# dschleef/schroedinger

Measured on AMD Instinct MI355X. Metric: Mpix/s IIWT+OBMC decode, 2160p s16, higher is better.
Workload: dtype s16

## Files before the change

### schroedinger_amd/csrc/iiwt_reg.hip

```cpp

#include "schro_hip_internal.h"
#include "iiwt_steps.h"

namespace schro {
namespace {

#define IWT_LOAD8(p) gload < u32x2 > (p)



__device__ __forceinline__ void
coh_store16 (char *p, u32x4 o)
{
  __hip_atomic_store ((SCHRO_GLOBAL uint64_t *) p, (uint64_t) o.x | ((uint64_t) o.y << 32), __ATOMIC_RELAXED, __HIP_MEMORY_SCOPE_AGENT);
  __hip_atomic_store ((SCHRO_GLOBAL uint64_t *) (p + 8), (uint64_t) o.z | ((uint64_t) o.w << 32), __ATOMIC_RELAXED, __HIP_MEMORY_SCOPE_AGENT);
}

typedef short s16x2 __attribute__ ((ext_vector_type (2)));
typedef uint32_t P;

constexpr int kRegRP = 12;
constexpr int kRegUC = 4 * 62;
constexpr int kRegThreads = 256;

// ... 263 lines not shown
  constexpr Step st = filter_step (F, K);
  constexpr int NT = kind_ntaps (st.kind);
  const P y = st.target ? row[0] : row[1];
  P p = lane_prev (y), n = lane_next (y);
  if constexpr (HEDGE) {
    p = is_first ? __builtin_amdgcn_perm (y, y, 0x01000100u) : p;
    n = is_last ? __builtin_amdgcn_perm (y, y, 0x03020302u) : n;
  }
  const P W[6] = { 0u, p, y, n, 0u, 0u };
  P s[NT];
  gather_taps < F, K, 0, 0, NT > (W, s);
  if (st.target)
    row[1] = lift_apply_pk < F, K > (row[1], s);
  else
    row[0] = lift_apply_pk < F, K > (row[0], s);
}

template < int F, bool HEDGE >
__device__ __forceinline__ void
l1_row (P (&row)[2], bool is_first, bool is_last, P & o0, P & o1)
{
  hstep2 < F, 0, HEDGE > (row, is_first, is_last);
  hstep2 < F, 1, HEDGE > (row, is_first, is_last);
  if constexpr (filter_nsteps (F) == 4) {
    hstep2 < F, 2, HEDGE > (row, is_first, is_last);
    hstep2 < F, 3, HEDGE > (row, is_first, is_last);
  }
  constexpr int SH = filter_shift (F);
  const P a = out_round_pk < SH > (row[0]), b = out_round_pk < SH > (row[1]);
  o0 = __builtin_amdgcn_perm (b, a, 0x05040100u);
  o1 = __builtin_amdgcn_perm (b, a, 0x07060302u);
}

template < int F, int RP, int LO, int HI, int LO1, int HI1, bool HEDGE >
__device__ __forceinline__ void
l1_phase (const IwtJob & job, int r0, int c0, int lane, bool is_first, bool is_last, P (&E)[RP][4])
{
  constexpr int H = filter_halo (F), RP1 = RP / 2 + 2 * H;
  static_assert (H % 2 == 0, "level 1 inside level 0 needs an even tile origin");
  P E1[RP1][2], O1[RP1][2];
  const int nr1 = job.h >> 2, nc1 = job.w >> 2;
  const int q0 = (r0 >> 1) - H;
  const uint32_t voff = (uint32_t) clampi ((c0 >> 1) + 2 * lane, 0, nc1 - 2) * 2u;
  constexpr Rng le = load_rows < F, RP1, LO1, HI1 > (0), lo = load_rows < F, RP1, LO1, HI1 > (1);
#pragma unroll
  for (int k = 0; k < RP1; k++) {
    const int r = clampi (q0 + k, 0, nr1 - 1);
    if (k >= le.lo && k <= le.hi) {
      E1[k][0] = gload < uint32_t > ((const char *) job.l1_sb[0] + (size_t) r * job.l1_sb_stride[0] + voff);
      E1[k][1] = gload < uint32_t > ((const char *) job.l1_sb[1] + (size_t) r * job.l1_sb_stride[1] + voff);
    }
    if (k >= lo.lo && k <= lo.hi) {
      O1[k][0] = gload < uint32_t > ((const char *) job.l1_sb[2] + (size_t) r * job.l1_sb_stride[2] + voff);
      O1[k][1] = gload < uint32_t > ((const char *) job.l1_sb[3] + (size_t) r * job.l1_sb_stride[3] + voff);
    }
  }
  vstep < F, 0, RP1, LO1, HI1 > (E1, O1);
  vstep < F, 1, RP1, LO1, HI1 > (E1, O1);
  if constexpr (filter_nsteps (F) == 4) {
    vstep < F, 2, RP1, LO1, HI1 > (E1, O1);
    vstep < F, 3, RP1, LO1, HI1 > (E1, O1);
  }
  constexpr Rng need = load_rows < F, RP, LO, HI > (0);
#pragma unroll
  for (int i = H; i < RP1 - H; i++) {
    const int k = 2 * (i - H);
    if (k >= need.lo && k <= need.hi)
      l1_row < F, HEDGE > (E1[i], is_first, is_last, E[k][0], E[k][1]);
    if (k + 1 >= need.lo && k + 1 <= need.hi)
      l1_row < F, HEDGE > (O1[i], is_first, is_last, E[k + 1][0], E[k + 1][1]);
  }
}

struct NoWait {
  struct Seen { };
  __device__ __forceinline__ Seen ask () const { return Seen (); }
  __device__ __forceinline__ void settle (Seen) const { }
};

template < int F, int RP, int LO, int HI, bool HEDGE, int COH = 0, typename WAIT = NoWait, int LO1 = 0, int HI1 = -1 >
__device__ __forceinline__ void
reg_tile (const IwtJob & job, int r0, int c0, int nr, int nc, int lane, WAIT wait = WAIT ())
{
  constexpr int H = filter_halo (F);
  P E[RP][4], O[RP][4];

  const int cl = c0 + 4 * lane;
  const uint32_t voff = (uint32_t) clampi (cl, 0, nc - 4) * 2u;
  constexpr Rng le = load_rows < F, RP, LO, HI > (0), lo = load_rows < F, RP, LO, HI > (1);
  const int l_lo = (max (0, -c0) + 3) >> 2, l_hi = min (63, ((nc - c0) >> 2) - 1);
  const bool is_first = lane == l_lo, is_last = lane == l_hi;
  if constexpr ((COH & 8) != 0) {
    l1_phase < F, RP, LO, HI, LO1, HI1, HEDGE > (job, r0, c0, lane, is_first, is_last, E);
    __builtin_amdgcn_sched_barrier (0);
  }
  const auto seen = wait.ask ();
#pragma unroll
  for (int k = 0; k < RP; k++) {
    const int r = clampi (r0 + k, 0, nr - 1);
    if (k >= le.lo && k <= le.hi) {
      const u32x2 hl = IWT_LOAD8 ((const char *) job.sb[1] + (size_t) r * job.sb_stride[1] + voff);
      E[k][2] = hl.x;
      E[k][3] = hl.y;
    }
    if (k >= lo.lo && k <= lo.hi) {
      const u32x2 lh = IWT_LOAD8 ((const char *) job.sb[2] + (size_t) r * job.sb_stride[2] + voff);
      const u32x2 hh = IWT_LOAD8 ((const char *) job.sb[3] + (size_t) r * job.sb_stride[3] + voff);
      O[k][0] = lh.x;
      O[k][1] = lh.y;
      O[k][2] = hh.x;
      O[k][3] = hh.y;
    }
  }
  wait.settle (seen);
  if constexpr ((COH & 8) == 0) {
#pragma unroll
    for (int k = 0; k < RP; k++) {
      const int r = clampi (r0 + k, 0, nr - 1);
      if (k >= le.lo && k <= le.hi) {
        const u32x2 ll = IWT_LOAD8 ((const char *) job.sb[0] + (size_t) r * job.sb_stride[0] + voff);
        E[k][0] = ll.x;
        E[k][1] = ll.y;
      }
    }
  }

  vstep < F, 0, RP, LO, HI > (E, O);
  vstep < F, 1, RP, LO, HI > (E, O);
  if constexpr (filter_nsteps (F) == 4) {
    vstep < F, 2, RP, LO, HI > (E, O);
    vstep < F, 3, RP, LO, HI > (E, O);
  }

  constexpr int LH = (COH & 8) != 0 ? l1_lane_halo (F) : 1;
  const bool store_lane = lane >= max (l_lo, LH) && lane <= min (l_hi, 63 - LH);
  if constexpr ((COH & 4) != 0) {
    const int x = 2 * cl, y0 = 2 * (r0 + H);
    const int nx = store_lane ? clampi (job.out_w - x, 0, 8) : 0;
    const bool full = nx == 8;
    const bool any_ragged = __builtin_amdgcn_readfirstlane ((int) (__ballot (nx > 0 && nx < 8) != 0)) != 0;
    const int xa = nx > 0 ? x : 0;
    char *dst = (char *) job.dst + (size_t) y0 *job.dst_stride + xa;
    const bool has_pred = job.pred != nullptr;
    const uint8_t *pp = job.pred + xa;
    const u32x2 k128 = (u32x2) { 0x80808080u, 0x80808080u };
    auto fetch = [&](int i, int odd) {
      const int row = min (y0 + 2 * (i - H) + odd, job.out_h - 1);
      return has_pred ? __builtin_nontemporal_load ((const SCHRO_GLOBAL u32x2 *) (pp + (size_t) row * job.pred_stride)) : k128;
    };
    constexpr int NPAIR = RP - 2 * H;
    constexpr int AHEAD = cmin (NPAIR, 4), RAMP = 2;
    u32x2 pr[NPAIR][2];
    __builtin_amdgcn_sched_barrier (0);
#pragma unroll
    for (int j = 0; j < AHEAD; j++) {
      pr[j][0] = fetch (H + j, 0);
      pr[j][1] = fetch (H + j, 1);
    }
    __builtin_amdgcn_sched_barrier (0);
#pragma unroll
    for (int i = H; i < RP - H; i++) {
      const int j = i - H;
      const int y = y0 + 2 * j;
      const Combine c0 = { pr[j][0], y < job.out_h, full, any_ragged, nx }, c1 = { pr[j][1], y + 1 < job.out_h, full, any_ragged, nx };
      finish_row < F, HEDGE, COH > (E[i], is_first, is_last, store_lane, dst, c0);
      finish_row < F, HEDGE, COH > (O[i], is_first, is_last, store_lane, dst + job.dst_stride, c1);
      dst += 2 * (size_t) job.dst_stride;
#pragma unroll
      for (int t = 0; t < RAMP; t++) {
        const int nj = AHEAD + RAMP * j + t;
        if (nj < NPAIR) {
          pr[nj][0] = fetch (H + nj, 0);
          pr[nj][1] = fetch (H + nj, 1);
        }
      }
      __builtin_amdgcn_sched_barrier (0);
    }
  } else {
    char *dst = (char *) job.dst + (size_t) (2 * (r0 + H)) * job.dst_stride + (size_t) cl * 4;
    const Combine none = { (u32x2) { 0u, 0u }, false, false, false, 0 };
#pragma unroll
    for (int i = H; i < RP - H; i++) {
      finish_row < F, HEDGE, COH > (E[i], is_first, is_last, store_lane, dst, none);
      finish_row < F, HEDGE, COH > (O[i], is_first, is_last, store_lane, dst + job.dst_stride, none);
      dst += 2 * (size_t) job.dst_stride;
    }
  }
}

template < int F, int RP, int N, int COH, typename WAIT >
__device__ __forceinline__ void
reg_tile_bottom (int nout, const IwtJob & job, int r0, int c0, int nr, int nc, int lane, WAIT wait)
{
  if constexpr (N >= 1) {
    if (nout == N)
      reg_tile < F, RP, 0, RP - 1 - N, true, COH, WAIT > (job, r0, c0, nr, nc, lane, wait);
    else
      reg_tile_bottom < F, RP, N - 1, COH, WAIT > (nout, job, r0, c0, nr, nc, lane, wait);
  }
}

template < int F, int RP >
__device__ __forceinline__ int
reg_tile_r0 (int ty, int nr)
{
  constexpr int H = filter_halo (F), UR = RP - 2 * H;
  int r0 = ty * UR - H;
  if (r0 + H + UR > nr)
    r0 = nr - UR - H;
  return r0;
}

template < int F, int RP, int COH, typename WAIT = NoWait >
__device__ __forceinline__ void
reg_tile_at (const IwtJob & job, int tx, int ty, int lane, WAIT wait = WAIT ())
{
  constexpr int H = filter_halo (F);
  const int nr = job.h >> 1, nc = job.w >> 1;
  const int r0 = reg_tile_r0 < F, RP > (ty, nr);
  const int nout = max (0, r0 + RP - nr);
  const int c0 = tx * kRegUC - 4;
  const bool hedge = c0 < 0 || c0 + 256 > nc;
  if (r0 < 0) {
    reg_tile < F, RP, H, RP - 1, true, COH, WAIT > (job, r0, c0, nr, nc, lane, wait);
  } else if (nout == 0) {
    if (!hedge)
      reg_tile < F, RP, 0, RP - 1, false, COH, WAIT > (job, r0, c0, nr, nc, lane, wait);
    else
      reg_tile < F, RP, 0, RP - 1, true, COH, WAIT > (job, r0, c0, nr, nc, lane, wait);
  } else {
    reg_tile_bottom < F, RP, H, COH, WAIT > (nout, job, r0, c0, nr, nc, lane, wait);
  }
}

template < int F, int RP, int LO, int HI, bool HEDGE, int COH, int N1 >
__device__ __forceinline__ void
reg_tile_l1_n1 (int n1, const IwtJob & job, int r0, int c0, int nr, int nc, int lane)
{
  constexpr int RP1 = RP / 2 + 2 * filter_halo (F);
  if constexpr (N1 >= 1) {
    if (n1 == N1)
      reg_tile < F, RP, LO, HI, HEDGE, COH, NoWait, 0, RP1 - 1 - N1 > (job, r0, c0, nr, nc, lane);
    else
      reg_tile_l1_n1 < F, RP, LO, HI, HEDGE, COH, N1 - 1 > (n1, job, r0, c0, nr, nc, lane);
  } else {
    reg_tile < F, RP, LO, HI, HEDGE, COH, NoWait, 0, RP1 - 1 > (job, r0, c0, nr, nc, lane);
  }
}

template < int F, int RP, int COH, int N >
__device__ __forceinline__ void
reg_tile_l1_bottom (int nout, const IwtJob & job, int r0, int c0, int nr, int nc, int lane)
{
  constexpr int H = filter_halo (F), RP1 = RP / 2 + 2 * H;
  if constexpr (N >= 1) {
    if constexpr (N % 2 == 0) {
      if (nout == N) {
        reg_tile < F, RP, 0, RP - 1 - N, true, COH, NoWait, 0, RP1 - 1 - H - N / 2 > (job, r0, c0, nr, nc, lane);
        return;
      }
    }
    reg_tile_l1_bottom < F, RP, COH, N - 1 > (nout, job, r0, c0, nr, nc, lane);
  }
}

template < int F, int RP, int COH >
__device__ __forceinline__ void
reg_tile_l1_at (const IwtJob & job, int tx, int ty, int lane)
{
  constexpr int H = filter_halo (F), RP1 = RP / 2 + 2 * H, LH = l1_lane_halo (F);
  const int nr = job.h >> 1, nc = job.w >> 1;
  const int r0 = reg_tile_r0 < F, RP > (ty, nr);
  const int nout = max (0, r0 + RP - nr);
  const int c0 = tx * (4 * (64 - 2 * LH)) - 4 * LH;
  const bool hedge = c0 < 0 || c0 + 256 > nc;
  if (r0 < 0) {
    reg_tile < F, RP, H, RP - 1, true, COH, NoWait, H + H / 2, RP1 - 1 > (job, r0, c0, nr, nc, lane);
  } else if (nout == 0) {
    const int n1 = max (0, (r0 + RP - nr) / 2 + H);
    if (!hedge)
      reg_tile_l1_n1 < F, RP, 0, RP - 1, false, COH, H > (n1, job, r0, c0, nr, nc, lane);
    else
      reg_tile_l1_n1 < F, RP, 0, RP - 1, true, COH, H > (n1, job, r0, c0, nr, nc, lane);
  } else {
    reg_tile_l1_bottom < F, RP, COH, H > (nout, job, r0, c0, nr, nc, lane);
  }
}

#define IIWT_REG_WAVES(F, RP) (((F) == 3 || (F) == 4) && (RP) == 12 ? 3 : 4)
#define IIWT_REG_WAVES_M(F, RP, MODE) (((MODE) & 8) != 0 ? 3 : (MODE) == 4 && (RP) == 12 ? 4 : IIWT_REG_WAVES (F, RP))
template < int F, int RP, int MODE >
__global__ __launch_bounds__ (kRegThreads) __attribute__ ((amdgpu_waves_per_eu (IIWT_REG_WAVES_M (F, RP, MODE), IIWT_REG_WAVES_M (F, RP, MODE))))
void iiwt_reg_kernel (const IwtJob * __restrict__ jobs, int njobs, int total_tiles)
{
  const int wg = xcd_tile_id (blockIdx.x, gridDim.x);
  const int tile = __builtin_amdgcn_readfirstlane (wg * (kRegThreads / 64) + (threadIdx.x >> 6));
  if (tile >= total_tiles)
    return;
  const int lane = threadIdx.x & 63;
  const IwtJob job = jobs[find_job (jobs, njobs, tile)];
  const int t = tile - job.tile_base;
  if constexpr ((MODE & 8) != 0)
    reg_tile_l1_at < F, RP, MODE > (job, t % job.tiles_x, t / job.tiles_x, lane);
  else
    reg_tile_at < F, RP, MODE > (job, t % job.tiles_x, t / job.tiles_x, lane);
}

constexpr int
small_rp (int f)
{
  return 4 + 2 * filter_halo (f);
}

constexpr int kChainPolls = 1 << 22;

struct ChainWait {
  const uint32_t *c;
  int n;
  uint32_t want;
  uint32_t *gave_up;
  uint32_t epoch;
  struct Seen {
    uint32_t v0, v1, v2;
  };
  __device__ __forceinline__ Seen ask () const
  {
    Seen s = { want, want, want };
    if (n > 0)
      s.v0 = __hip_atomic_load (c, __ATOMIC_RELAXED, __HIP_MEMORY_SCOPE_AGENT);
    if (n > 1)
      s.v1 = __hip_atomic_load (c + 1, __ATOMIC_RELAXED, __HIP_MEMORY_SCOPE_AGENT);
    if (n > 2)
      s.v2 = __hip_atomic_load (c + 2, __ATOMIC_RELAXED, __HIP_MEMORY_SCOPE_AGENT);
    return s;
  }
  __device__ __forceinline__ void settle (Seen s) const
// ... 39 lines not shown
    wait.gave_up = gave_up;
    wait.epoch = epoch;
  }
  if (job.ctr >= 0) {
    if (job.small)
      reg_tile_at < F, small_rp (F), 2, ChainWait > (job, tx, ty, lane, wait);
    else
      reg_tile_at < F, kRegRP, 2, ChainWait > (job, tx, ty, lane, wait);
    __builtin_amdgcn_s_waitcnt (0x0f70);
    if (lane == 0)
      __hip_atomic_fetch_add (&ctrl[job.ctr + ty], 1u, __ATOMIC_RELAXED, __HIP_MEMORY_SCOPE_AGENT);
  } else {
    if (job.small)
      reg_tile_at < F, small_rp (F), 0, ChainWait > (job, tx, ty, lane, wait);
    else
      reg_tile_at < F, kRegRP, 0, ChainWait > (job, tx, ty, lane, wait);
  }
}

template < int F >
int
launch_chain (hipStream_t stream, const IwtJob * d_jobs, const uint32_t * d_order, int n_tiles, uint32_t * ctrl, uint32_t run,
    uint32_t * gave_up, uint32_t epoch)
{
  const int wgs = (n_tiles + kRegThreads / 64 - 1) / (kRegThreads / 64);
  SCHRO_LAUNCH ((iiwt_chain_kernel < F >), dim3 (wgs), dim3 (kRegThreads), 0, stream, d_jobs, d_order, n_tiles, ctrl, run,
      gave_up, epoch);
  hipError_t e = hipGetLastError ();
  if (e != hipSuccess)
    return set_error (SCHRO_HIP_EDEVICE, "iiwt (chain form) launch: %s", hipGetErrorString (e));
  return 0;
}

template < int F >
int
launch_reg (hipStream_t stream, const IwtJob * d_jobs, int njobs, int total_tiles, bool small, bool combine, bool l1)
{
  const int wgs = (total_tiles + kRegThreads / 64 - 1) / (kRegThreads / 64);
  if constexpr (l1_built (F)) {
    if (l1) {
      if (small)
        return set_error (SCHRO_HIP_EINVAL, "iiwt (register form): level 1 inside level 0 takes the large tile only");
      if (combine)
        SCHRO_LAUNCH ((iiwt_reg_kernel < F, kRegRP, 12 >), dim3 (wgs), dim3 (kRegThreads), 0, stream, d_jobs, njobs,
            total_tiles);
      else
        SCHRO_LAUNCH ((iiwt_reg_kernel < F, kRegRP, 8 >), dim3 (wgs), dim3 (kRegThreads), 0, stream, d_jobs, njobs,
            total_tiles);
      hipError_t e = hipGetLastError ();
      if (e != hipSuccess)
        return set_error (SCHRO_HIP_EDEVICE, "iiwt (register form, level 1 inside) launch: %s", hipGetErrorString (e));
      return 0;
    }
  } else if (l1) {
    return set_error (SCHRO_HIP_EINVAL, "iiwt (register form): level 1 inside level 0 is not built for filter %d", F);
  }
  if (small && combine)
    SCHRO_LAUNCH ((iiwt_reg_kernel < F, small_rp (F), 4 >), dim3 (wgs), dim3 (kRegThreads), 0, stream,
        d_jobs, njobs, total_tiles);
  else if (combine)
    SCHRO_LAUNCH ((iiwt_reg_kernel < F, kRegRP, 4 >), dim3 (wgs), dim3 (kRegThreads), 0, stream, d_jobs,
        njobs, total_tiles);
  else if (small)
    SCHRO_LAUNCH ((iiwt_reg_kernel < F, small_rp (F), 0 >), dim3 (wgs), dim3 (kRegThreads), 0, stream,
        d_jobs, njobs, total_tiles);
  else
    SCHRO_LAUNCH ((iiwt_reg_kernel < F, kRegRP, 0 >), dim3 (wgs), dim3 (kRegThreads), 0, stream, d_jobs,
        njobs, total_tiles);
  hipError_t e = hipGetLastError ();
  if (e != hipSuccess)
    return set_error (SCHRO_HIP_EDEVICE, "iiwt (register form) launch: %s", hipGetErrorString (e));
  return 0;
}

}

bool
iiwt_reg_supported (int filter, int bpp)
{
  return bpp == 2 && filter != 5 && filter >= 0 && filter <= 6;
}

void
iiwt_reg_geometry (int filter, int small, int *useful_cols, int *useful_row_pairs, int *min_row_pairs)
{
  const int rp = small ? small_rp (filter) : kRegRP;
  *useful_cols = kRegUC;
  *useful_row_pairs = rp - 2 * filter_halo (filter);
  *min_row_pairs = rp - filter_halo (filter);
}

bool
iiwt_reg_l1_supported (int filter)
{
  return iiwt_reg_supported (filter, 2) && l1_built (filter);
}

void
iiwt_reg_l1_geometry (int filter, int *useful_cols, int *useful_row_pairs, int *min_row_pairs)
{
  *useful_cols = 4 * (64 - 2 * l1_lane_halo (filter));
  *useful_row_pairs = kRegRP - 2 * filter_halo (filter);
  *min_row_pairs = kRegRP + 2 * filter_halo (filter);
}

int
launch_iiwt_chain (hipStream_t stream, const IwtJob * d_jobs, const uint32_t * d_order, int n_tiles, uint32_t * ctrl,
    uint32_t run, uint32_t * gave_up, uint32_t epoch, int filter)
{
#ifdef SCHRO_HIP_EXPERIMENTS
  switch (filter) {
    case 0: return launch_chain < 0 > (stream, d_jobs, d_order, n_tiles, ctrl, run, gave_up, epoch);
    case 1: return launch_chain < 1 > (stream, d_jobs, d_order, n_tiles, ctrl, run, gave_up, epoch);
    case 2: return launch_chain < 2 > (stream, d_jobs, d_order, n_tiles, ctrl, run, gave_up, epoch);
    case 3: return launch_chain < 3 > (stream, d_jobs, d_order, n_tiles, ctrl, run, gave_up, epoch);
    case 4: return launch_chain < 4 > (stream, d_jobs, d_order, n_tiles, ctrl, run, gave_up, epoch);
    case 6: return launch_chain < 6 > (stream, d_jobs, d_order, n_tiles, ctrl, run, gave_up, epoch);
  }
  return set_error (SCHRO_HIP_EINVAL, "iiwt (chain form): filter %d not built", filter);
#else
  (void) stream, (void) d_jobs, (void) d_order, (void) n_tiles, (void) ctrl, (void) run, (void) gave_up, (void) epoch, (void) filter;
  return set_error (SCHRO_HIP_EUNSUPPORTED, "the chain form of the register wavelet is built into the experiments library only");
#endif
}

int
launch_iiwt_reg (hipStream_t stream, const IwtJob * d_jobs, int njobs, int total_tiles, int filter,
    int small, int combine, int l1_inline)
{
  switch (filter) {
    case 0: return launch_reg < 0 > (stream, d_jobs, njobs, total_tiles, small, combine, l1_inline);
    case 1: return launch_reg < 1 > (stream, d_jobs, njobs, total_tiles, small, combine, l1_inline);
    case 2: return launch_reg < 2 > (stream, d_jobs, njobs, total_tiles, small, combine, l1_inline);
    case 3: return launch_reg < 3 > (stream, d_jobs, njobs, total_tiles, small, combine, l1_inline);
    case 4: return launch_reg < 4 > (stream, d_jobs, njobs, total_tiles, small, combine, l1_inline);
    case 6: return launch_reg < 6 > (stream, d_jobs, njobs, total_tiles, small, combine, l1_inline);
  }
  return set_error (SCHRO_HIP_EINVAL, "iiwt (register form): filter %d not built", filter);
}

}
```

### schroedinger_amd/csrc/plane_iiwt.cpp

```cpp

#include "schro_hip_internal.h"

#include <cstdio>
#include <cstdlib>
#include <cstring>
#include <algorithm>

using namespace schro;

extern "C" {


static int
iiwt_fused_group (SchroHipContext * ctx, const SchroHipIwtPlane * planes, int nplanes, int depth,
    int filter, int bpp, int fb, int nl, const std::vector < size_t > &scratch_off,
    const std::vector < int >&scratch_stride, int uc, int ur)
{
  const size_t jsz = iiwt_fused_job_size ();
  std::vector < char >fj (jsz * nplanes);
  int tile_base = 0;
  for (int p = 0; p < nplanes; p++) {
    const SchroHipIwtPlane & pl = planes[p];
    const int top = fb + nl;
    const void *ll = pl.src;
// ... 320 lines not shown
      }
    } else {
      j.dst = (char *) ctx->scratch_ref () + scratch_off[(size_t) p * depth + level];
      j.dst_stride = scratch_stride[(size_t) p * depth + level];
    }
    j.w = w;
    j.h = h;
    int nc = w / 2;
    int vl = 8 / bpp;
    bool src_al = (nc % vl) == 0 && nc >= vl;
    for (int s = 0; s < 4; s++)
      src_al = src_al && (((uintptr_t) j.sb[s] | (uintptr_t) j.sb_stride[s]) & 7) == 0;
    bool dst_al = (((uintptr_t) j.dst | (uintptr_t) j.dst_stride) & (j.pad2 ? 7 : 15)) == 0;
    j.flags = (src_al ? 1 : 0) | (dst_al ? 2 : 0);
    j.ctr = -1;
    *src_al_out = src_al;
    *dst_al_out = dst_al;
    return j;
  };
  auto level_is_small = [&](int level) {
    long tiles = 0;
    for (int p = 0; p < nplanes; p++)
      tiles += (long) div_up ((planes[p].width >> level) / 2, ruc) * div_up ((planes[p].height >> level) / 2, rur);
    const char *env = SCHRO_ENV ("SCHRO_HIP_IIWT_SMALL");
    const char *envb = SCHRO_ENV ("SCHRO_HIP_IIWT_SMALL_BELOW");
    return env ? atoi (env) != 0 : tiles < (envb ? atol (envb) : 2048);
  };

  const bool chain_on = SCHRO_ENV ("SCHRO_HIP_IIWT_CHAIN") && atoi (SCHRO_ENV ("SCHRO_HIP_IIWT_CHAIN")) != 0;
  const bool l1_on = use_reg && depth >= 2 && iiwt_reg_l1_supported (filter) && !chain_on
      && !(SCHRO_ENV ("SCHRO_HIP_IIWT_FUSE") && atoi (SCHRO_ENV ("SCHRO_HIP_IIWT_FUSE")) != 0)
      && !(SCHRO_ENV ("SCHRO_HIP_IIWT_L1_INLINE") && atoi (SCHRO_ENV ("SCHRO_HIP_IIWT_L1_INLINE")) == 0)
      && !level_is_small (0);
  int l1uc = 0, l1ur = 0, l1rmin = 0;
  if (l1_on)
    iiwt_reg_l1_geometry (filter, &l1uc, &l1ur, &l1rmin);
  std::vector < char >l1_inline (nplanes, 0);
  auto plane_l1_inline = [&](int p) {
    if (!l1_on)
      return false;
    bool a0, d0, a1, d1;
    const IwtJob j0 = level_job (p, 0, &a0, &d0), j1 = level_job (p, 1, &a1, &d1);
    int uc1, ur1, rmin1;
    iiwt_reg_geometry (filter, level_is_small (1), &uc1, &ur1, &rmin1);
    return (!planes[p].combine || j0.pad2) && a0 && d0 && (j0.w / 2) % 4 == 0 && j0.h / 2 >= l1rmin
        && a1 && (j1.w / 2) % 4 == 0 && j1.h / 2 >= rmin1;
  };
  size_t total = 0;
  bool any_ll = false;
  for (int p = 0; p < nplanes; p++) {
    const SchroHipIwtPlane & pl = planes[p];
    SCHRO_HIP_REQUIRE (pl.src && pl.dst, "iiwt_batch: plane %d has a NULL pointer", p);
    SCHRO_HIP_REQUIRE (pl.width > 0 && pl.height > 0 && pl.width % (1 << depth) == 0
        && pl.height % (1 << depth) == 0,
        "iiwt_batch: plane %d size %dx%d is not a multiple of 2^depth", p, pl.width, pl.height);
    SCHRO_HIP_REQUIRE (pl.combine >= 0 && pl.combine <= 2 && (pl.combine == 0 || (pl.out_width > 0 && pl.out_height > 0
                && pl.out_width <= pl.width && pl.out_height <= pl.height)) && (pl.combine != 1 || (pl.pred && pl.pred_stride >= pl.out_width)),
        "iiwt_batch: plane %d: combine %d needs out_width x out_height inside the transform (and a prediction plane for 1)", p, pl.combine);
    SCHRO_HIP_REQUIRE (pl.src_stride >= pl.width * bpp && pl.dst_stride >= (pl.combine ? pl.out_width : pl.width * bpp),
        "iiwt_batch: plane %d stride too small", p);
    SCHRO_HIP_REQUIRE (!pl.ll || (pl.ll_stride >= (pl.width >> depth) * bpp && ((uintptr_t) pl.ll | (uintptr_t) pl.ll_stride) % bpp == 0),
        "iiwt_batch: plane %d: the LL plane's stride %d does not hold %d samples", p, pl.ll_stride, pl.width >> depth);
    any_ll |= pl.ll != nullptr;
    {
      const char *s0 = (const char *) pl.src, *s1 = s0 + (size_t) pl.src_stride * pl.height;
      const char *d0 = (const char *) pl.dst, *d1 = d0 + (size_t) pl.dst_stride * (pl.combine ? pl.out_height : pl.height);
      SCHRO_HIP_REQUIRE (s1 <= d0 || d1 <= s0, "iiwt_batch: plane %d src and dst overlap", p);
    }
    if (pl.combine) {
// ... 165 lines not shown
          rjobs.push_back (j);
        }
      } else if (j.pad2) {
        return set_error (SCHRO_HIP_EINVAL, "iiwt_batch: plane %d: the combine form was promised a register tile it cannot have", p);
      } else {
        j.tiles_x = div_up (nc, uc);
        j.tile_base = tile_base;
        tile_base += j.tiles_x * div_up (nr, ur);
        jobs.push_back (j);
      }
    }
    void *d_rjobs = nullptr, *d_jobs = nullptr, *d_hjobs = nullptr, *d_cjobs = nullptr, *d_r1jobs = nullptr, *d_c1jobs = nullptr;
    int r = 0;
    if (!rjobs.empty ())
      r = push_args (ctx, rjobs.data (), sizeof (IwtJob) * rjobs.size (), &d_rjobs);
    if (!r && !r1jobs.empty ())
      r = push_args (ctx, r1jobs.data (), sizeof (IwtJob) * r1jobs.size (), &d_r1jobs);
    if (!r && !c1jobs.empty ())
      r = push_args (ctx, c1jobs.data (), sizeof (IwtJob) * c1jobs.size (), &d_c1jobs);
    if (!r && !cjobs.empty ())
      r = push_args (ctx, cjobs.data (), sizeof (IwtJob) * cjobs.size (), &d_cjobs);
    if (!r && !hjobs.empty ())
      r = push_args (ctx, hjobs.data (), sizeof (IwtJob) * hjobs.size (), &d_hjobs);
    if (!r && !jobs.empty ())
      r = push_args (ctx, jobs.data (), sizeof (IwtJob) * jobs.size (), &d_jobs);
    if (r)
      return r;
    ProfileScope ps (ctx, level == 0 ? SCHRO_HIP_KERNEL_IIWT_FINEST : SCHRO_HIP_KERNEL_IIWT_COARSE);
    if (d_rjobs)
      r = launch_iiwt_reg (ctx->stream, (const IwtJob *) d_rjobs, (int) rjobs.size (), rtile_base, filter, small, 0);
    if (!r && d_cjobs)
      r = launch_iiwt_reg (ctx->stream, (const IwtJob *) d_cjobs, (int) cjobs.size (), ctile_base, filter, small, 1);
    if (!r && d_r1jobs)
      r = launch_iiwt_reg (ctx->stream, (const IwtJob *) d_r1jobs, (int) r1jobs.size (), r1tile_base, filter, 0, 0, 1);
    if (!r && d_c1jobs)
      r = launch_iiwt_reg (ctx->stream, (const IwtJob *) d_c1jobs, (int) c1jobs.size (), c1tile_base, filter, 0, 1, 1);
    if (!r && d_hjobs)
      r = launch_iiwt_haar (ctx->stream, (const IwtJob *) d_hjobs, (int) hjobs.size (), htile_base, filter);
    if (!r && d_jobs)
      r = launch_iiwt_level (ctx->stream, (const IwtJob *) d_jobs, (int) jobs.size (), tile_base, filter, bpp);
    if (r)
      return r;
  }
  return iiwt_combine_temps (ctx, planes, nplanes, depth, bpp, scratch_off, scratch_stride);
}

}
```

### schroedinger_amd/csrc/schro_hip_internal.h

```cpp
#pragma once

#include <hip/hip_runtime.h>
#include <hip/hip_ext.h>
#include <cstdint>
#include <cstddef>
#include <vector>

#include "schro_hip.h"

#ifdef SCHRO_HIP_DRY
#include "schro_hip_dry.h"
#endif

#ifdef SCHRO_HIP_EXPERIMENTS
#define SCHRO_ENV(name) getenv (name)
#else
#define SCHRO_ENV(name) ((const char *) nullptr)
#endif

namespace schro {

int set_error (int code, const char *fmt, ...);
int set_status (int code, const char *fmt, ...);

// ... 509 lines not shown
  }
  if (njobs > 64) {
    const int idx = (lo >> 6) + lane;
    const bool le = idx < n64 && gload < int > (first + njobs + idx) <= bid;
    lo += (__popcll (__ballot (le)) - 1) * 64;
  }
  const int idx = lo + lane;
  const bool le = idx < njobs && gload < int > (first + idx) <= bid;
  return __builtin_amdgcn_readfirstlane (lo + __popcll (__ballot (le)) - 1);
}
#endif

int launch_iiwt_level (hipStream_t stream, const IwtJob * d_jobs, int njobs,
    int total_tiles, int filter, int bpp);

size_t iiwt_fused_job_size (void);
int iiwt_fused_max_levels (int filter, int bpp);
void iiwt_fused_job_fill (void *job, const void *src, int src_stride, int bpp, int nl,
    const void *ll, int ll_stride, void *dst, int dst_stride, int w, int h, int tiles_x,
    int tile_base);
int launch_iiwt_fused (hipStream_t stream, const void *d_jobs, int njobs, int total_tiles,
    int filter, int bpp, int nl);
bool iiwt_haar_supported (int filter, int bpp);
bool iiwt_haar_job_ok (const IwtJob & j);
void iiwt_haar_geometry (int *cols, int *rows);
int launch_iiwt_haar (hipStream_t stream, const IwtJob * d_jobs, int njobs, int total_tiles, int filter);
bool iiwt_haar3_job_ok (const void *src, int src_stride, const void *dst, int dst_stride, int w, int h);
void iiwt_haar3_geometry (int *blocks_x, int *blocks_y);
int launch_iiwt_haar3 (hipStream_t stream, const IwtJob * d_jobs, int njobs, int total_tiles, int filter);
bool iiwt_reg_supported (int filter, int bpp);
void iiwt_reg_geometry (int filter, int small, int *useful_cols, int *useful_row_pairs,
    int *min_row_pairs);
int launch_iiwt_reg (hipStream_t stream, const IwtJob * d_jobs, int njobs, int total_tiles,
    int filter, int small, int combine, int l1_inline = 0);
bool iiwt_reg_l1_supported (int filter);
void iiwt_reg_l1_geometry (int filter, int *useful_cols, int *useful_row_pairs, int *min_row_pairs);
int launch_iiwt_chain (hipStream_t stream, const IwtJob * d_jobs, const uint32_t * d_order, int n_tiles, uint32_t * ctrl,
    uint32_t run, uint32_t * gave_up, uint32_t epoch, int filter);
void iiwt_tile_geometry (int filter, int bpp, int *useful_cols,
    int *useful_row_pairs);
void iwt_fwd_tile_geometry (int filter, int bpp, int *useful_cols, int *useful_row_pairs);
int launch_iwt_fwd_level (hipStream_t stream, const IwtFwdJob * d_jobs, int njobs, int total_tiles, int filter, int bpp);
void downsample_tile_geometry (int *cols, int *rows);
int launch_downsample (hipStream_t stream, const DownsampleJob * d_jobs, int njobs, int total_tiles);
size_t scan_lds_bytes (int bw, int bh, int sw, int sh);
size_t scan_lds_limit ();
int launch_metric_scan (hipStream_t stream, const ScanPicture * d_pics, const ScanJob * d_scans, int nscans, size_t lds_per_wave);
int launch_rough_hint (hipStream_t stream, const RoughChain * d_chains, int nchains, size_t lds_per_wave);
int launch_convert (hipStream_t stream, const ConvertJob * d_jobs, int njobs,
    int total_tiles, int bpp);
void convert_tile_geometry (int *tw, int *th);
int launch_pack (hipStream_t stream, const PackJob * d_jobs, int njobs, int total_tiles);
int launch_shift_right (hipStream_t stream, const ConvertJob * d_jobs, int njobs, int total_tiles, int bpp, int shift);
int launch_add (hipStream_t stream, const ConvertJob * d_jobs, int njobs, int total_tiles, int src_bpp, bool subtract);
void pack_tile_geometry (int *groups_x, int *rows);
int launch_upsample (hipStream_t stream, const UpsampleJob * d_jobs,
    int njobs, int total_tiles, int persist_grid);
void upsample_tile_geometry (int *tw, int *th);
int launch_slices (hipStream_t stream, const SliceJob * d_jobs, int njobs, const SliceParams & P, int bpp, int arith,
    bool aligned16);
bool dc_skew_ok (const DcJob * jobs, int njobs, int bpp);
int launch_dc_predict (hipStream_t stream, const DcJob * d_jobs, int njobs, int max_rows, int bpp,
    unsigned long long *edge, int edge_pitch, uint32_t epoch, uint32_t * gave_up);
int dc_edge_for (SchroHipContext * ctx, int njobs, int max_rows, int max_w, unsigned long long **edge,
    int *edge_pitch, uint32_t * epoch);
int dc_gave_up (SchroHipContext * ctx);
int pred_overflow_poll (SchroHipContext * ctx);
int pred_overflow_claim (SchroHipContext * ctx, uint32_t epoch);
}
// ... 203 lines not shown
```

Before: 203,000.

## Defer level-1 lifting past level-0 loads and shrink L1-inline tile to 10 row pairs

Splits the level-1-inside phase into a load-issue step and a lifting step so the level-1 coefficient loads (and optionally early prediction fetches) can overlap the level-0 subband loads. It adds selectable load orders, and the default variant uses a 10-row-pair tile with 4 waves per EU instead of 12 rows at 3 waves. Smaller tiles raise occupancy but recompute more halo rows per useful output, and keeping level-1 values live longer adds register pressure.

After: 198,000. 2.5% lower.

```diff
diff --git a/schroedinger_amd/csrc/iiwt_reg.hip b/schroedinger_amd/csrc/iiwt_reg.hip
--- a/schroedinger_amd/csrc/iiwt_reg.hip
+++ b/schroedinger_amd/csrc/iiwt_reg.hip
@@ -319,13 +319,19 @@
   o1 = __builtin_amdgcn_perm (b, a, 0x07060302u);
 }
 
-template < int F, int RP, int LO, int HI, int LO1, int HI1, bool HEDGE >
-__device__ __forceinline__ void
-l1_phase (const IwtJob & job, int r0, int c0, int lane, bool is_first, bool is_last, P (&E)[RP][4])
-{
-  constexpr int H = filter_halo (F), RP1 = RP / 2 + 2 * H;
+constexpr int
+l1_region_rows (int f, int rp)
+{
+  return rp / 2 + 2 * filter_halo (f);
+}
+
+template < int F, int RP, int RP1, int LO1, int HI1 >
+__device__ __forceinline__ void
+l1_issue (const IwtJob & job, int r0, int c0, int lane, P (&E1)[RP1][2], P (&O1)[RP1][2])
+{
+  constexpr int H = filter_halo (F);
   static_assert (H % 2 == 0, "level 1 inside level 0 needs an even tile origin");
-  P E1[RP1][2], O1[RP1][2];
+  static_assert (RP1 == l1_region_rows (F, RP), "the level-1 region of the tile");
   const int nr1 = job.h >> 2, nc1 = job.w >> 2;
   const int q0 = (r0 >> 1) - H;
   const uint32_t voff = (uint32_t) clampi ((c0 >> 1) + 2 * lane, 0, nc1 - 2) * 2u;
@@ -342,6 +348,13 @@
       O1[k][1] = gload < uint32_t > ((const char *) job.l1_sb[3] + (size_t) r * job.l1_sb_stride[3] + voff);
     }
   }
+}
+
+template < int F, int RP, int RP1, int LO, int HI, int LO1, int HI1, bool HEDGE >
+__device__ __forceinline__ void
+l1_lift (bool is_first, bool is_last, P (&E1)[RP1][2], P (&O1)[RP1][2], P (&E)[RP][4])
+{
+  constexpr int H = filter_halo (F);
   vstep < F, 0, RP1, LO1, HI1 > (E1, O1);
   vstep < F, 1, RP1, LO1, HI1 > (E1, O1);
   if constexpr (filter_nsteps (F) == 4) {
@@ -365,20 +378,70 @@
   __device__ __forceinline__ void settle (Seen) const { }
 };
 
-template < int F, int RP, int LO, int HI, bool HEDGE, int COH = 0, typename WAIT = NoWait, int LO1 = 0, int HI1 = -1 >
+struct CombineLane {
+  int nx;
+  bool full, any_ragged;
+  char *dst;
+  const uint8_t *pp;
+  bool has_pred;
+  int y0, out_h, pred_stride;
+  __device__ __forceinline__ u32x2 fetch (int j, int odd) const
+  {
+    const int row = min (y0 + 2 * j + odd, out_h - 1);
+    return has_pred ? __builtin_nontemporal_load ((const SCHRO_GLOBAL u32x2 *) (pp + (size_t) row * pred_stride))
+        : (u32x2) { 0x80808080u, 0x80808080u };
+  }
+};
+
+__device__ __forceinline__ CombineLane
+combine_lane (const IwtJob & job, int cl, int y0, bool store_lane)
+{
+  CombineLane c;
+  const int x = 2 * cl;
+  c.nx = store_lane ? clampi (job.out_w - x, 0, 8) : 0;
+  c.full = c.nx == 8;
+  c.any_ragged = __builtin_amdgcn_readfirstlane ((int) (__ballot (c.nx > 0 && c.nx < 8) != 0)) != 0;
+  const int xa = c.nx > 0 ? x : 0;
+  c.dst = (char *) job.dst + (size_t) y0 *job.dst_stride + xa;
+  c.has_pred = job.pred != nullptr;
+  c.pp = job.pred + xa;
+  c.y0 = y0;
+  c.out_h = job.out_h;
+  c.pred_stride = job.pred_stride;
+  return c;
+}
+
+constexpr int
+l1_loads_pre (int l1_loads, int npair)
+{
+  return l1_loads == 2 ? npair : l1_loads == 1 ? cmin (npair, 2) : 0;
+}
+
+template < int F, int RP, int LO, int HI, bool HEDGE, int COH = 0, typename WAIT = NoWait, int LO1 = 0, int HI1 = -1, int L1_LOADS = 0 >
 __device__ __forceinline__ void
 reg_tile (const IwtJob & job, int r0, int c0, int nr, int nc, int lane, WAIT wait = WAIT ())
 {
   constexpr int H = filter_halo (F);
+  constexpr int RP1 = (COH & 8) != 0 ? l1_region_rows (F, RP) : 1;
+  constexpr int NPAIR = RP - 2 * H;
+  constexpr int PRE = (COH & 12) == 12 ? l1_loads_pre (L1_LOADS, NPAIR) : 0;
   P E[RP][4], O[RP][4];
+  P E1[RP1][2], O1[RP1][2];
+  u32x2 pr[NPAIR][2];
+  (void) E1, (void) O1, (void) pr;
 
   const int cl = c0 + 4 * lane;
   const uint32_t voff = (uint32_t) clampi (cl, 0, nc - 4) * 2u;
   constexpr Rng le = load_rows < F, RP, LO, HI > (0), lo = load_rows < F, RP, LO, HI > (1);
   const int l_lo = (max (0, -c0) + 3) >> 2, l_hi = min (63, ((nc - c0) >> 2) - 1);
   const bool is_first = lane == l_lo, is_last = lane == l_hi;
+  constexpr int LH = (COH & 8) != 0 ? l1_lane_halo (F) : 1;
+  const bool store_lane = lane >= max (l_lo, LH) && lane <= min (l_hi, 63 - LH);
   if constexpr ((COH & 8) != 0) {
-    l1_phase < F, RP, LO, HI, LO1, HI1, HEDGE > (job, r0, c0, lane, is_first, is_last, E);
+    l1_issue < F, RP, RP1, LO1, HI1 > (job, r0, c0, lane, E1, O1);
+    if constexpr (L1_LOADS == 0) {
+      l1_lift < F, RP, RP1, LO, HI, LO1, HI1, HEDGE > (is_first, is_last, E1, O1, E);
+    }
     __builtin_amdgcn_sched_barrier (0);
   }
   const auto seen = wait.ask ();
@@ -411,6 +474,18 @@
       }
     }
   }
+  if constexpr ((COH & 8) != 0 && L1_LOADS != 0) {
+    if constexpr (PRE > 0) {
+      const CombineLane cb = combine_lane (job, cl, 2 * (r0 + H), store_lane);
+#pragma unroll
+      for (int j = 0; j < PRE; j++) {
+        pr[j][0] = cb.fetch (j, 0);
+        pr[j][1] = cb.fetch (j, 1);
+      }
+    }
+    __builtin_amdgcn_sched_barrier (0);
+    l1_lift < F, RP, RP1, LO, HI, LO1, HI1, HEDGE > (is_first, is_last, E1, O1, E);
+  }
 
   vstep < F, 0, RP, LO, HI > (E, O);
   vstep < F, 1, RP, LO, HI > (E, O);
@@ -419,30 +494,17 @@
     vstep < F, 3, RP, LO, HI > (E, O);
   }
 
-  constexpr int LH = (COH & 8) != 0 ? l1_lane_halo (F) : 1;
-  const bool store_lane = lane >= max (l_lo, LH) && lane <= min (l_hi, 63 - LH);
   if constexpr ((COH & 4) != 0) {
-    const int x = 2 * cl, y0 = 2 * (r0 + H);
-    const int nx = store_lane ? clampi (job.out_w - x, 0, 8) : 0;
-    const bool full = nx == 8;
-    const bool any_ragged = __builtin_amdgcn_readfirstlane ((int) (__ballot (nx > 0 && nx < 8) != 0)) != 0;
-    const int xa = nx > 0 ? x : 0;
-    char *dst = (char *) job.dst + (size_t) y0 *job.dst_stride + xa;
-    const bool has_pred = job.pred != nullptr;
-    const uint8_t *pp = job.pred + xa;
-    const u32x2 k128 = (u32x2) { 0x80808080u, 0x80808080u };
-    auto fetch = [&](int i, int odd) {
-      const int row = min (y0 + 2 * (i - H) + odd, job.out_h - 1);
-      return has_pred ? __builtin_nontemporal_load ((const SCHRO_GLOBAL u32x2 *) (pp + (size_t) row * job.pred_stride)) : k128;
-    };
-    constexpr int NPAIR = RP - 2 * H;
-    constexpr int AHEAD = cmin (NPAIR, 4), RAMP = 2;
-    u32x2 pr[NPAIR][2];
+    const CombineLane cb = combine_lane (job, cl, 2 * (r0 + H), store_lane);
+    const int y0 = cb.y0, nx = cb.nx;
+    const bool full = cb.full, any_ragged = cb.any_ragged;
+    char *dst = cb.dst;
+    constexpr int AHEAD = cmax (PRE, cmin (NPAIR, 4)), RAMP = 2;
     __builtin_amdgcn_sched_barrier (0);
 #pragma unroll
-    for (int j = 0; j < AHEAD; j++) {
-      pr[j][0] = fetch (H + j, 0);
-      pr[j][1] = fetch (H + j, 1);
+    for (int j = PRE; j < AHEAD; j++) {
+      pr[j][0] = cb.fetch (j, 0);
+      pr[j][1] = cb.fetch (j, 1);
     }
     __builtin_amdgcn_sched_barrier (0);
 #pragma unroll
@@ -457,8 +519,8 @@
       for (int t = 0; t < RAMP; t++) {
         const int nj = AHEAD + RAMP * j + t;
         if (nj < NPAIR) {
-          pr[nj][0] = fetch (H + nj, 0);
-          pr[nj][1] = fetch (H + nj, 1);
+          pr[nj][0] = cb.fetch (nj, 0);
+          pr[nj][1] = cb.fetch (nj, 1);
         }
       }
       __builtin_amdgcn_sched_barrier (0);
@@ -520,22 +582,22 @@
   }
 }
 
-template < int F, int RP, int LO, int HI, bool HEDGE, int COH, int N1 >
+template < int F, int RP, int LO, int HI, bool HEDGE, int COH, int L1_LOADS, int N1 >
 __device__ __forceinline__ void
 reg_tile_l1_n1 (int n1, const IwtJob & job, int r0, int c0, int nr, int nc, int lane)
 {
   constexpr int RP1 = RP / 2 + 2 * filter_halo (F);
   if constexpr (N1 >= 1) {
     if (n1 == N1)
-      reg_tile < F, RP, LO, HI, HEDGE, COH, NoWait, 0, RP1 - 1 - N1 > (job, r0, c0, nr, nc, lane);
+      reg_tile < F, RP, LO, HI, HEDGE, COH, NoWait, 0, RP1 - 1 - N1, L1_LOADS > (job, r0, c0, nr, nc, lane);
     else
-      reg_tile_l1_n1 < F, RP, LO, HI, HEDGE, COH, N1 - 1 > (n1, job, r0, c0, nr, nc, lane);
+      reg_tile_l1_n1 < F, RP, LO, HI, HEDGE, COH, L1_LOADS, N1 - 1 > (n1, job, r0, c0, nr, nc, lane);
   } else {
-    reg_tile < F, RP, LO, HI, HEDGE, COH, NoWait, 0, RP1 - 1 > (job, r0, c0, nr, nc, lane);
-  }
-}
-
-template < int F, int RP, int COH, int N >
+    reg_tile < F, RP, LO, HI, HEDGE, COH, NoWait, 0, RP1 - 1, L1_LOADS > (job, r0, c0, nr, nc, lane);
+  }
+}
+
+template < int F, int RP, int COH, int L1_LOADS, int N >
 __device__ __forceinline__ void
 reg_tile_l1_bottom (int nout, const IwtJob & job, int r0, int c0, int nr, int nc, int lane)
 {
@@ -543,15 +605,15 @@
   if constexpr (N >= 1) {
     if constexpr (N % 2 == 0) {
       if (nout == N) {
-        reg_tile < F, RP, 0, RP - 1 - N, true, COH, NoWait, 0, RP1 - 1 - H - N / 2 > (job, r0, c0, nr, nc, lane);
+        reg_tile < F, RP, 0, RP - 1 - N, true, COH, NoWait, 0, RP1 - 1 - H - N / 2, L1_LOADS > (job, r0, c0, nr, nc, lane);
         return;
       }
     }
-    reg_tile_l1_bottom < F, RP, COH, N - 1 > (nout, job, r0, c0, nr, nc, lane);
-  }
-}
-
-template < int F, int RP, int COH >
+    reg_tile_l1_bottom < F, RP, COH, L1_LOADS, N - 1 > (nout, job, r0, c0, nr, nc, lane);
+  }
+}
+
+template < int F, int RP, int COH, int L1_LOADS >
 __device__ __forceinline__ void
 reg_tile_l1_at (const IwtJob & job, int tx, int ty, int lane)
 {
@@ -562,22 +624,22 @@
   const int c0 = tx * (4 * (64 - 2 * LH)) - 4 * LH;
   const bool hedge = c0 < 0 || c0 + 256 > nc;
   if (r0 < 0) {
-    reg_tile < F, RP, H, RP - 1, true, COH, NoWait, H + H / 2, RP1 - 1 > (job, r0, c0, nr, nc, lane);
+    reg_tile < F, RP, H, RP - 1, true, COH, NoWait, H + H / 2, RP1 - 1, L1_LOADS > (job, r0, c0, nr, nc, lane);
   } else if (nout == 0) {
     const int n1 = max (0, (r0 + RP - nr) / 2 + H);
     if (!hedge)
-      reg_tile_l1_n1 < F, RP, 0, RP - 1, false, COH, H > (n1, job, r0, c0, nr, nc, lane);
+      reg_tile_l1_n1 < F, RP, 0, RP - 1, false, COH, L1_LOADS, H > (n1, job, r0, c0, nr, nc, lane);
     else
-      reg_tile_l1_n1 < F, RP, 0, RP - 1, true, COH, H > (n1, job, r0, c0, nr, nc, lane);
+      reg_tile_l1_n1 < F, RP, 0, RP - 1, true, COH, L1_LOADS, H > (n1, job, r0, c0, nr, nc, lane);
   } else {
-    reg_tile_l1_bottom < F, RP, COH, H > (nout, job, r0, c0, nr, nc, lane);
+    reg_tile_l1_bottom < F, RP, COH, L1_LOADS, H > (nout, job, r0, c0, nr, nc, lane);
   }
 }
 
 #define IIWT_REG_WAVES(F, RP) (((F) == 3 || (F) == 4) && (RP) == 12 ? 3 : 4)
-#define IIWT_REG_WAVES_M(F, RP, MODE) (((MODE) & 8) != 0 ? 3 : (MODE) == 4 && (RP) == 12 ? 4 : IIWT_REG_WAVES (F, RP))
-template < int F, int RP, int MODE >
-__global__ __launch_bounds__ (kRegThreads) __attribute__ ((amdgpu_waves_per_eu (IIWT_REG_WAVES_M (F, RP, MODE), IIWT_REG_WAVES_M (F, RP, MODE))))
+#define IIWT_REG_WAVES_M(F, RP, MODE, L1_LOADS) (((MODE) & 8) != 0 ? ((RP) <= 10 ? 4 : (L1_LOADS) == 2 ? 2 : 3) : (MODE) == 4 && (RP) == 12 ? 4 : IIWT_REG_WAVES (F, RP))
+template < int F, int RP, int MODE, int L1_LOADS = 0 >
+__global__ __launch_bounds__ (kRegThreads) __attribute__ ((amdgpu_waves_per_eu (IIWT_REG_WAVES_M (F, RP, MODE, L1_LOADS), IIWT_REG_WAVES_M (F, RP, MODE, L1_LOADS))))
 void iiwt_reg_kernel (const IwtJob * __restrict__ jobs, int njobs, int total_tiles)
 {
   const int wg = xcd_tile_id (blockIdx.x, gridDim.x);
@@ -588,7 +650,7 @@
   const IwtJob job = jobs[find_job (jobs, njobs, tile)];
   const int t = tile - job.tile_base;
   if constexpr ((MODE & 8) != 0)
-    reg_tile_l1_at < F, RP, MODE > (job, t % job.tiles_x, t / job.tiles_x, lane);
+    reg_tile_l1_at < F, RP, MODE, L1_LOADS > (job, t % job.tiles_x, t / job.tiles_x, lane);
   else
     reg_tile_at < F, RP, MODE > (job, t % job.tiles_x, t / job.tiles_x, lane);
 }
@@ -694,21 +756,63 @@
   return 0;
 }
 
+constexpr int kL1Variant = 5;
+constexpr int kL1Variants = 6;
+
+constexpr int
+l1_variant_rp (int v)
+{
+  return v >= 4 ? 10 : kRegRP;
+}
+
+constexpr int
+l1_variant_order (int v)
+{
+  return v == 3 ? 2 : v >= 4 ? v - 4 : v;
+}
+
+template < int F, int V >
+void
+launch_reg_l1 (hipStream_t stream, const IwtJob * d_jobs, int njobs, int total_tiles, int wgs, bool combine)
+{
+  constexpr int RP = l1_variant_rp (V), L1_LOADS = l1_variant_order (V);
+  const int lds = V == 3 ? 64 * 1024 : 0;
+  (void) RP, (void) L1_LOADS, (void) lds;
+  if (combine)
+    SCHRO_LAUNCH ((iiwt_reg_kernel < F, RP, 12, L1_LOADS >), dim3 (wgs), dim3 (kRegThreads), lds, stream, d_jobs, njobs,
+        total_tiles);
+  else
+    SCHRO_LAUNCH ((iiwt_reg_kernel < F, RP, 8, L1_LOADS >), dim3 (wgs), dim3 (kRegThreads), lds, stream, d_jobs, njobs,
+        total_tiles);
+}
+
 template < int F >
 int
-launch_reg (hipStream_t stream, const IwtJob * d_jobs, int njobs, int total_tiles, bool small, bool combine, bool l1)
+launch_reg (hipStream_t stream, const IwtJob * d_jobs, int njobs, int total_tiles, bool small, bool combine, bool l1, int l1_loads)
 {
   const int wgs = (total_tiles + kRegThreads / 64 - 1) / (kRegThreads / 64);
   if constexpr (l1_built (F)) {
     if (l1) {
       if (small)
         return set_error (SCHRO_HIP_EINVAL, "iiwt (register form): level 1 inside level 0 takes the large tile only");
-      if (combine)
-        SCHRO_LAUNCH ((iiwt_reg_kernel < F, kRegRP, 12 >), dim3 (wgs), dim3 (kRegThreads), 0, stream, d_jobs, njobs,
-            total_tiles);
-      else
-        SCHRO_LAUNCH ((iiwt_reg_kernel < F, kRegRP, 8 >), dim3 (wgs), dim3 (kRegThreads), 0, stream, d_jobs, njobs,
-            total_tiles);
+      if (l1_loads < 0)
+        l1_loads = kL1Variant;
+#ifdef SCHRO_HIP_EXPERIMENTS
+      switch (l1_loads) {
+        case 0: launch_reg_l1 < F, 0 > (stream, d_jobs, njobs, total_tiles, wgs, combine); break;
+        case 1: launch_reg_l1 < F, 1 > (stream, d_jobs, njobs, total_tiles, wgs, combine); break;
+        case 2: launch_reg_l1 < F, 2 > (stream, d_jobs, njobs, total_tiles, wgs, combine); break;
+        case 3: launch_reg_l1 < F, 3 > (stream, d_jobs, njobs, total_tiles, wgs, combine); break;
+        case 4: launch_reg_l1 < F, 4 > (stream, d_jobs, njobs, total_tiles, wgs, combine); break;
+        case 5: launch_reg_l1 < F, 5 > (stream, d_jobs, njobs, total_tiles, wgs, combine); break;
+        default:
+          return set_error (SCHRO_HIP_EINVAL, "iiwt (register form): no load order %d of the level-1-inside tile", l1_loads);
+      }
+#else
+      if (l1_loads != kL1Variant)
+        return set_error (SCHRO_HIP_EUNSUPPORTED, "iiwt (register form): load order %d is built into the experiments library only", l1_loads);
+      launch_reg_l1 < F, kL1Variant > (stream, d_jobs, njobs, total_tiles, wgs, combine);
+#endif
       hipError_t e = hipGetLastError ();
       if (e != hipSuccess)
         return set_error (SCHRO_HIP_EDEVICE, "iiwt (register form, level 1 inside) launch: %s", hipGetErrorString (e));
@@ -759,11 +863,12 @@
 }
 
 void
-iiwt_reg_l1_geometry (int filter, int *useful_cols, int *useful_row_pairs, int *min_row_pairs)
-{
+iiwt_reg_l1_geometry (int filter, int l1_loads, int *useful_cols, int *useful_row_pairs, int *min_row_pairs)
+{
+  const int rp = l1_variant_rp (l1_loads < 0 || l1_loads >= kL1Variants ? kL1Variant : l1_loads);
   *useful_cols = 4 * (64 - 2 * l1_lane_halo (filter));
-  *useful_row_pairs = kRegRP - 2 * filter_halo (filter);
-  *min_row_pairs = kRegRP + 2 * filter_halo (filter);
+  *useful_row_pairs = rp - 2 * filter_halo (filter);
+  *min_row_pairs = rp + 2 * filter_halo (filter);
 }
 
 int
@@ -788,15 +893,15 @@
 
 int
 launch_iiwt_reg (hipStream_t stream, const IwtJob * d_jobs, int njobs, int total_tiles, int filter,
-    int small, int combine, int l1_inline)
+    int small, int combine, int l1_inline, int l1_loads)
 {
   switch (filter) {
-    case 0: return launch_reg < 0 > (stream, d_jobs, njobs, total_tiles, small, combine, l1_inline);
-    case 1: return launch_reg < 1 > (stream, d_jobs, njobs, total_tiles, small, combine, l1_inline);
-    case 2: return launch_reg < 2 > (stream, d_jobs, njobs, total_tiles, small, combine, l1_inline);
-    case 3: return launch_reg < 3 > (stream, d_jobs, njobs, total_tiles, small, combine, l1_inline);
-    case 4: return launch_reg < 4 > (stream, d_jobs, njobs, total_tiles, small, combine, l1_inline);
-    case 6: return launch_reg < 6 > (stream, d_jobs, njobs, total_tiles, small, combine, l1_inline);
+    case 0: return launch_reg < 0 > (stream, d_jobs, njobs, total_tiles, small, combine, l1_inline, l1_loads);
+    case 1: return launch_reg < 1 > (stream, d_jobs, njobs, total_tiles, small, combine, l1_inline, l1_loads);
+    case 2: return launch_reg < 2 > (stream, d_jobs, njobs, total_tiles, small, combine, l1_inline, l1_loads);
+    case 3: return launch_reg < 3 > (stream, d_jobs, njobs, total_tiles, small, combine, l1_inline, l1_loads);
+    case 4: return launch_reg < 4 > (stream, d_jobs, njobs, total_tiles, small, combine, l1_inline, l1_loads);
+    case 6: return launch_reg < 6 > (stream, d_jobs, njobs, total_tiles, small, combine, l1_inline, l1_loads);
   }
   return set_error (SCHRO_HIP_EINVAL, "iiwt (register form): filter %d not built", filter);
 }
diff --git a/schroedinger_amd/csrc/plane_iiwt.cpp b/schroedinger_amd/csrc/plane_iiwt.cpp
--- a/schroedinger_amd/csrc/plane_iiwt.cpp
+++ b/schroedinger_amd/csrc/plane_iiwt.cpp
@@ -376,9 +376,10 @@
       && !(SCHRO_ENV ("SCHRO_HIP_IIWT_FUSE") && atoi (SCHRO_ENV ("SCHRO_HIP_IIWT_FUSE")) != 0)
       && !(SCHRO_ENV ("SCHRO_HIP_IIWT_L1_INLINE") && atoi (SCHRO_ENV ("SCHRO_HIP_IIWT_L1_INLINE")) == 0)
       && !level_is_small (0);
+  const int l1_loads = SCHRO_ENV ("SCHRO_HIP_IIWT_L1_LOADS") ? atoi (SCHRO_ENV ("SCHRO_HIP_IIWT_L1_LOADS")) : -1;
   int l1uc = 0, l1ur = 0, l1rmin = 0;
   if (l1_on)
-    iiwt_reg_l1_geometry (filter, &l1uc, &l1ur, &l1rmin);
+    iiwt_reg_l1_geometry (filter, l1_loads, &l1uc, &l1ur, &l1rmin);
   std::vector < char >l1_inline (nplanes, 0);
   auto plane_l1_inline = [&](int p) {
     if (!l1_on)
@@ -610,9 +611,9 @@
     if (!r && d_cjobs)
       r = launch_iiwt_reg (ctx->stream, (const IwtJob *) d_cjobs, (int) cjobs.size (), ctile_base, filter, small, 1);
     if (!r && d_r1jobs)
-      r = launch_iiwt_reg (ctx->stream, (const IwtJob *) d_r1jobs, (int) r1jobs.size (), r1tile_base, filter, 0, 0, 1);
+      r = launch_iiwt_reg (ctx->stream, (const IwtJob *) d_r1jobs, (int) r1jobs.size (), r1tile_base, filter, 0, 0, 1, l1_loads);
     if (!r && d_c1jobs)
-      r = launch_iiwt_reg (ctx->stream, (const IwtJob *) d_c1jobs, (int) c1jobs.size (), c1tile_base, filter, 0, 1, 1);
+      r = launch_iiwt_reg (ctx->stream, (const IwtJob *) d_c1jobs, (int) c1jobs.size (), c1tile_base, filter, 0, 1, 1, l1_loads);
     if (!r && d_hjobs)
       r = launch_iiwt_haar (ctx->stream, (const IwtJob *) d_hjobs, (int) hjobs.size (), htile_base, filter);
     if (!r && d_jobs)
diff --git a/schroedinger_amd/csrc/schro_hip_internal.h b/schroedinger_amd/csrc/schro_hip_internal.h
--- a/schroedinger_amd/csrc/schro_hip_internal.h
+++ b/schroedinger_amd/csrc/schro_hip_internal.h
@@ -565,9 +565,9 @@
 void iiwt_reg_geometry (int filter, int small, int *useful_cols, int *useful_row_pairs,
     int *min_row_pairs);
 int launch_iiwt_reg (hipStream_t stream, const IwtJob * d_jobs, int njobs, int total_tiles,
-    int filter, int small, int combine, int l1_inline = 0);
+    int filter, int small, int combine, int l1_inline = 0, int l1_loads = -1);
 bool iiwt_reg_l1_supported (int filter);
-void iiwt_reg_l1_geometry (int filter, int *useful_cols, int *useful_row_pairs, int *min_row_pairs);
+void iiwt_reg_l1_geometry (int filter, int l1_loads, int *useful_cols, int *useful_row_pairs, int *min_row_pairs);
 int launch_iiwt_chain (hipStream_t stream, const IwtJob * d_jobs, const uint32_t * d_order, int n_tiles, uint32_t * ctrl,
     uint32_t run, uint32_t * gave_up, uint32_t epoch, int filter);
 void iiwt_tile_geometry (int filter, int bpp, int *useful_cols,
```
